# wuqianliang/Diff-Reg

Hardware: AMD Instinct MI355X
Metric: scene-pairs/sec @ 20 denoise steps (N=M=256); IR/FMR parity vs ref (higher is better)
Workload: dtype f32; 1 GPU; cfg2: 3DMatch N=M=256, C=432, 20 denoise steps, max_condition_num=200 (warp active), 256 independent B=1 pairs per pass per GPU as 2 concurrent batch(es), one HIP-graph replay each on its own stream; pairs_per_pass_per_gpu=256, streams=2, denoise_steps=20, N=256, M=256, graph=True, parallelism=pairs sharded over 1 GPU(s)

## Files before the change

diff-reg_amd/csrc/loop.hip:

```cpp
#include "loop_common.h"

namespace dr {

struct LayerWs {
    float *qkv, *att, *mrg, *msg, *hid, *g2;
    size_t T;
    static size_t carve(Carver& c, LayerWs& w, size_t T, int C) {
        w.T = T;
        w.qkv = c.take<float>(T * 3 * C);
        w.att = c.take<float>(T * C);
        w.mrg = c.take<float>(T * C);
        w.msg = c.take<float>(T * C);
        w.hid = c.take<float>(T * 2 * C);
        w.g2 = c.take<float>(T * C);
        return c.off;
    }
};

struct PrepackLayer {
    PgW qkv, merge, mlp0, mlp2;
    const float *lnB1, *lnB2;
};
struct Prepack {
    static constexpr int MAXL = 16;
// ... 56 lines not shown
            if (rc) return rc;
        }
        return pp.head.sub == 2 ? pgemm16w_pack_weights_block(W.src_proj, C, C, C, C, pp.head, 0, st)
                                : pgemm_pack_weights_block(W.src_proj, C, C, C, C, pp.head, 0, st);
    }
};

struct PlanesWs {
    bool on;
    Tok feat0, fa, fb, tgt_l0;
    char *att_img, *msg_img, *hid_img;
    float *att_bnd, *msg_bnd, *hid_bnd;
    char *qkv_img, *kvc_img;
    float *qkv_bnd, *kvc_bnd;
    float* grp_x;
    float* csT;
    size_t qkv_stride;
    size_t side_C, side_att, side_hid;
    void* own_pack;
    float* xk_buf; unsigned* xk_flags; mutable unsigned xk_epoch; unsigned* status;
    static size_t img_bytes(int PN, int PM, int K) { return plane_image_bytes(PN, K) + plane_image_bytes(PM, K); }
    static void carve(Carver& c, PlanesWs& w, const dr_loop_config& cfg, int P, int N, int M) {
        const int C = cfg.C, PN = P * N, PM = P * M, T = PN + PM;
        w.on = planes_wanted(cfg.flags, Prepack::supported(cfg), T);
        if (!w.on) return;
        const int dp = (C / cfg.H + 15) / 16 * 16;
        w.side_C = plane_image_bytes(PN, C); w.side_att = plane_image_bytes(PN, cfg.H * dp); w.side_hid = plane_image_bytes(PN, 2 * C);
        Tok* toks[4] = {&w.feat0, &w.fa, &w.fb, &w.tgt_l0};
        for (Tok* t : toks) { t->f32 = nullptr; t->img = c.take<char>(img_bytes(PN, PM, C)); t->bnd = c.take<float>(T); }
        w.att_img = c.take<char>(img_bytes(PN, PM, cfg.H * dp)); w.att_bnd = c.take<float>(T);
        w.msg_img = c.take<char>(img_bytes(PN, PM, C)); w.msg_bnd = c.take<float>(T);
        w.hid_img = c.take<char>(img_bytes(PN, PM, 2 * C)); w.hid_bnd = c.take<float>(T);
        w.qkv_stride = (img_bytes(PN, PM, cfg.H * dp) + 255) & ~(size_t)255;
        w.qkv_img = c.take<char>(3 * w.qkv_stride); w.qkv_bnd = c.take<float>(3 * (size_t)T);
        w.kvc_img = c.take<char>(2 * w.qkv_stride); w.kvc_bnd = c.take<float>(2 * (size_t)T);
        w.grp_x = c.take<float>(2 * (size_t)P);
        w.csT = c.take<float>((size_t)T * C);
        w.own_pack = c.take<char>(Prepack::carve(nullptr, cfg, nullptr));
        const bool xk = (T + 63) / 64 + 2 <= PG_XK_MAX_RB;
        w.xk_buf = xk ? c.take<float>(pgemm_xk_buf_bytes(pgemm_bn(C)) / 4) : nullptr;
        w.xk_flags = xk ? c.take<unsigned>(pgemm_xk_flag_bytes() / 4) : nullptr;
        w.xk_epoch = 0; w.status = nullptr;
    }
};

static int layer_call(const dr_layer_weights& W, int C, int H, int P, const float* xin, int xr0, int xrows,
                      const float* yin, int yr0, int yrows, const float* cosT, const float* sinT,
                      const uint8_t* tokmask, const Family& f1, const Family* f2, const LayerWs& ws, float* out,
                      hipStream_t st, const float* kv_cached = nullptr, float* kv_store = nullptr, const float* xq_in = nullptr,
                      const float* yk_in = nullptr) {
    const int halfC = C / 2, d = C / H;
    const bool rotary = cosT != nullptr;
    const float* const qin = xq_in ? xq_in : xin;
    const float* const kin = yk_in ? yk_in : yin;
    GemmBatch g;
    memset(&g, 0, sizeof(g));
    auto proj = [&](GemmProblem& p, const float* in, int r0, int rows, const float* Wm, int coloff, bool rot) {
// ... 67 lines not shown
struct PlCtx {
    const Prepack* pp; const PlanesWs* pw; const LayerWs* lw;
    int C, H, P, N, M;
    const float *cosT, *sinT;
    const uint8_t* tokmask;
    int attn_f16;
};
static void xk_assign(const PlanesWs& pw, int C, PgProblem& p, size_t& next, size_t units) {
    if (!pw.xk_buf || next + units > (size_t)PG_XK_MAX_RB) return;
    p.xk_buf = pw.xk_buf + next * (pgemm_xk_buf_bytes(pgemm_bn(C)) / 4 / PG_XK_MAX_RB); p.xk_flags = pw.xk_flags + next * 2; p.xk_cap = (int)units;
    p.xk_epoch = pw.xk_epoch + 1; p.xk_status = pw.status;
    next += units;
}
static size_t xk_wide_units(const PgProblem& p) { return (size_t)(p.rows + 127) / 128 * p.nblk * 2; }

static int layer_call_planes(const PlCtx& X, const dr_layer_weights& W, int l, const Tok& xin, int xs, const Tok& yin, int ys,
                             const Tok& out, const Family& f1, const Family* f2, hipStream_t st, const float* kv_cached = nullptr,
                             float* kv_store = nullptr) {
    const int C = X.C, H = X.H, PN = X.P * X.N, PM = X.P * X.M, halfC = C / 2, d = C / H, nC = C / 16, dp = X.pp->dp;
    const PrepackLayer& L = X.pp->L[l];
    const PlanesWs& pw = *X.pw;
    auto r0 = [&](int side) { return side == SIDE_TGT ? PN : 0; };
    auto nrows = [&](int side) { return side == SIDE_TGT ? PM : PN; };
    auto at = [&](char* img, size_t side_off, int side) { return img + (side == SIDE_TGT ? side_off : 0); };
    PgBatch g;
    size_t xk_next = 0;
    auto reset = [&]() { memset(&g, 0, sizeof(g)); xk_next = 0; };
    auto add = [&]() -> PgProblem& { return g.p[g.n++]; };
    auto for_sides = [&](int mask, auto fn) { for (int side = 1; side <= 2; ++side) if (mask & side) fn(side); };
    auto xk = [&](PgProblem& p, size_t units) { xk_assign(pw, C, p, xk_next, units); };
    int rc;
    bool rc_ok = true;

    const int T = PN + PM, Cq = H * dp, nq = Cq / 16;
    const bool cached = kv_cached != nullptr;
    char* const kv_img = kv_store ? pw.kvc_img : pw.qkv_img + pw.qkv_stride;
    float* const kv_bnd = kv_store ? pw.kvc_bnd : pw.qkv_bnd + T;
    const bool grp_inline = X.N % 128 == 0 && X.M % 128 == 0 && env_knob("DR_LOOP_GRP_INLINE", 1) != 0;
    if (!cached && !grp_inline) {
        for (int side = 1; side <= 2 && rc_ok; ++side)
            if (ys & side) rc_ok = launch_group_max(yin.bnd + r0(side), X.P, side == SIDE_TGT ? X.M : X.N, pw.grp_x + (side == SIDE_TGT ? X.P : 0), st) == DR_OK;
        if (!rc_ok) return DR_ELAUNCH;
    }
    auto proj = [&](const Tok& tin, int side, int b0, int nblk, char* img, float* bnd, int rotm, int grpm) {
        PgProblem& p = add();
        p.A0 = at(tin.img, pw.side_C, side); p.bnd0 = tin.bnd + r0(side); p.nc0 = nC;
        p.W = pgw_blocks(L.qkv, b0, C); p.nblk = nblk; p.rows = nrows(side); p.C = Cq; p.k_alg = C; p.mode = PG_PLANES;
        p.rot_mask = rotm; p.rot_C = C; p.rot_piece_len = d; p.rot_piece_pad = dp; p.scale = 1.f;
        p.cosT = X.cosT + (size_t)r0(side) * halfC; p.sinT = X.sinT + (size_t)r0(side) * halfC;
        p.csT = X.pw->csT + (size_t)r0(side) * halfC * 2;
        p.pimg = at(img, pw.side_att, side); p.p_nct = nq; p.pbnd = bnd + r0(side);
        p.pimg_blk_stride = (long long)pw.qkv_stride; p.pbnd_blk_stride = T;
        p.grp_bnd = grp_inline ? nullptr : pw.grp_x; p.grp_mask = grpm; p.grp_first = side == SIDE_TGT ? X.P : 0; p.grp_rows = side == SIDE_TGT ? X.M : X.N;
        if (p.W.sub == 2) xk(p, xk_wide_units(p));
    };
    reset();
    if (kv_store) {
        for_sides(ys, [&](int side) { proj(yin, side, 1, 2, kv_img, kv_bnd, 1, 3); });
        ++pw.xk_epoch;
        return launch_pgemm(g, st);
    }
    const bool self = xs == ys && xin.img == yin.img && !cached;
    if (self) {
        for_sides(xs, [&](int side) { proj(xin, side, 0, 3, pw.qkv_img, pw.qkv_bnd, 3, 6); });
    } else {
        for_sides(xs, [&](int side) { proj(xin, side, 0, 1, pw.qkv_img, pw.qkv_bnd, 1, 0); });
        if (!cached) for_sides(ys, [&](int side) { proj(yin, side, 1, 2, kv_img, kv_bnd, 1, 3); });
    }
    ++pw.xk_epoch;
    rc = launch_pgemm(g, st);
    if (rc) return rc;

    AttnArgs a;
    memset(&a, 0, sizeof(a));
    a.H = H; a.d = d;
    a.qmask = X.tokmask; a.kmask = X.tokmask;
    a.nseg = X.P; a.q0 = f1.q0; a.qstride = f1.Lq; a.Lq = f1.Lq; a.k0 = f1.k0; a.kstride = f1.Lk; a.Lk = f1.Lk;
    if (f2) { a.nseg2 = X.P; a.q0b = f2->q0; a.qstrideb = f2->Lq; a.Lqb = f2->Lq; a.k0b = f2->k0; a.kstrideb = f2->Lk; a.Lkb = f2->Lk; }
    a.scale = 1.0f / sqrtf((float)d);
    a.pimg[0] = pw.att_img; a.pimg[1] = pw.att_img + pw.side_att; a.p_split = PN; a.p_nct = nq; a.p_dp = dp;
    a.pbnd = pw.att_bnd;
    {
        const char* kimg = cached ? pw.kvc_img : pw.qkv_img + pw.qkv_stride;
        const float* kb = cached ? pw.kvc_bnd : pw.qkv_bnd + T;
        a.qimg[0] = pw.qkv_img; a.qimg[1] = pw.qkv_img + pw.side_att;
        a.kimg[0] = kimg; a.kimg[1] = kimg + pw.side_att;
        a.vimg[0] = kimg + pw.qkv_stride; a.vimg[1] = kimg + pw.qkv_stride + pw.side_att;
        a.qbnd = pw.qkv_bnd; a.kgb = kb; a.vgb = kb + T;
        a.f16_single = X.attn_f16;
    }
    rc = launch_attention(a, st);
    if (rc) return rc;

    reset();
    for_sides(xs, [&](int side) {
        PgProblem& p = add();
        p.A0 = at(pw.att_img, pw.side_att, side); p.bnd0 = pw.att_bnd + r0(side); p.nc0 = H * dp / 16;
        p.W = L.merge; p.nblk = 1; p.rows = nrows(side); p.C = C; p.mode = PG_LN; p.k_alg = C;
        p.gamma = W.norm1_w; p.beta = W.norm1_b; p.lnB = L.lnB1;
        p.pimg = at(pw.msg_img, pw.side_C, side); p.p_nct = nC; p.pbnd = pw.msg_bnd + r0(side);
        xk(p, (size_t)(p.rows + 63) / 64);
    });
    ++pw.xk_epoch;
// ... 23 lines not shown
        xk(p, (size_t)(p.rows + 63) / 64);
    });
    ++pw.xk_epoch;
    return launch_pgemm(g, st);
}

struct DenoiseWs {
    LayerWs lw;
    float *fa, *fb, *cosT, *sinT, *proj, *sim;
    float *tgt_l0, *kv_l1;
    PlanesWs pl;
    const Prepack* pp;
    static void carve(Carver& c, DenoiseWs& w, const dr_loop_config& cfg, int P, int N, int M) {
        const int C = cfg.C;
        const size_t T = (size_t)P * (N + M);
        LayerWs::carve(c, w.lw, T, C);
        PlanesWs::carve(c, w.pl, cfg, P, N, M);
        w.tgt_l0 = c.take<float>(T * C);
        w.kv_l1 = c.take<float>(T * 2 * C);
        w.fa = c.take<float>(T * C);
        w.fb = c.take<float>(T * C);
        w.cosT = c.take<float>(T * (C / 2));
        w.sinT = c.take<float>(T * (C / 2));
        w.proj = c.take<float>(T * C);
        w.sim = c.take<float>((size_t)P * N * M);
        if (w.pl.on) { w.pl.fa.f32 = w.fa; w.pl.fb.f32 = w.fb; w.pl.tgt_l0.f32 = w.tgt_l0; }
    }
};

static int fill_tgt_cache(const dr_loop_config& cfg, const dr_loop_weights& w, int P, int N, int M, const float* feat0,
                          const uint8_t* tokmask, DenoiseWs& ws, hipStream_t st) {
    const int C = cfg.C, H = cfg.H, PN = P * N, PM = P * M;
    const Family self_t{PN, M, PN, M};
    if (ws.pl.on) {
        const PlCtx X{ws.pp, &ws.pl, &ws.lw, C, H, P, N, M, ws.cosT, ws.sinT, tokmask, (cfg.flags & DR_LOOP_ATTN_F16) ? 1 : 0};
        int rc = layer_call_planes(X, w.layers[0], 0, ws.pl.feat0, SIDE_TGT, ws.pl.feat0, SIDE_TGT, ws.pl.tgt_l0, self_t, nullptr, st);
        if (rc || cfg.n_layers < 2) return rc;
        return layer_call_planes(X, w.layers[1], 1, ws.pl.tgt_l0, 0, ws.pl.tgt_l0, SIDE_TGT, ws.pl.tgt_l0, self_t, nullptr, st, nullptr, ws.kv_l1);
    }
    int rc = layer_call(w.layers[0], C, H, P, feat0, PN, PM, feat0, PN, PM, ws.cosT, ws.sinT, tokmask, self_t, nullptr, ws.lw,
                        ws.tgt_l0, st);
    if (rc || cfg.n_layers < 2) return rc;
    return layer_call(w.layers[1], C, H, P, nullptr, 0, 0, ws.tgt_l0, PN, PM, ws.cosT, ws.sinT, tokmask, self_t, nullptr, ws.lw,
                      nullptr, st, nullptr, ws.kv_l1);
}

static int denoiser_and_sim(const dr_loop_config& cfg, const dr_loop_weights& w, int P, int N, int M, const float* feat0,
                            const uint8_t* tokmask, DenoiseWs& ws, const float** final_feats, hipStream_t st,
                            bool use_cache = false) {
    const int C = cfg.C, H = cfg.H, T = P * (N + M), PN = P * N, PM = P * M;
    auto head = [&](const float* feats) {
        return gemm1(feats, C, w.src_proj, nullptr, ws.proj, C, T, C, C, EPI_ROTARY, 1.0f / sqrtf((float)C), nullptr, st, ws.cosT, ws.sinT, C);
    };
    auto sim = [&]() {
        return gemm1(ws.proj, C, ws.proj + (size_t)PN * C, nullptr, ws.sim, M, N, M, C, EPI_NONE, 1.f, nullptr, st, nullptr, nullptr, 0, P,
                     (long long)N * C, (long long)M * C, (long long)N * M);
    };
    if (ws.pl.on) {
        const PlCtx X{ws.pp, &ws.pl, &ws.lw, C, H, P, N, M, ws.cosT, ws.sinT, tokmask, (cfg.flags & DR_LOOP_ATTN_F16) ? 1 : 0};
        const Family self_s{0, N, 0, N}, self_t{PN, M, PN, M}, cross_s{0, N, PN, M}, cross_t{PN, M, 0, N};
        const Tok* cur = &ws.pl.feat0;
        const Tok* bufs[2] = {&ws.pl.fa, &ws.pl.fb};
        int which = 0;
        for (int l = 0; l < cfg.n_layers; ++l) {
            const Tok* nxt = bufs[which];
            int rc;
            if (use_cache && l == 0) {
                nxt = &ws.pl.tgt_l0;
                rc = layer_call_planes(X, w.layers[0], 0, *cur, SIDE_SRC, *cur, SIDE_SRC, *nxt, self_s, nullptr, st);
                if (rc) return rc;
                cur = nxt;
                continue;
            } else if (l % 2 == 0) {
                rc = layer_call_planes(X, w.layers[l], l, *cur, SIDE_BOTH, *cur, SIDE_BOTH, *nxt, self_s, &self_t, st);
                if (rc) return rc;
            } else {
                rc = layer_call_planes(X, w.layers[l], l, *cur, SIDE_SRC, *cur, SIDE_TGT, *nxt, cross_s, nullptr, st,
                                       (use_cache && l == 1) ? ws.kv_l1 : nullptr);
                if (rc) return rc;
                rc = layer_call_planes(X, w.layers[l], l, *cur, SIDE_TGT, *nxt, SIDE_SRC, *nxt, cross_t, nullptr, st);
                if (rc) return rc;
            }
            cur = nxt;
            which ^= 1;
        }
        *final_feats = cur->f32;
        if (env_knob("DR_HEAD_F32", 0)) {
            const int rc = head(cur->f32);
            return rc ? rc : sim();
        }
        PgBatch g;
        memset(&g, 0, sizeof(g));
        size_t xk_next = 0;
        for (int side = 1; side <= 2; ++side) {
            PgProblem& p = g.p[g.n++];
// ... 296 lines not shown
    DR_HIP_CHECK(hipMemcpyAsync(L.feat0, src_feats, PN * C * 4, hipMemcpyDeviceToDevice, st));
    DR_HIP_CHECK(hipMemcpyAsync(L.feat0 + PN * C, tgt_feats, PM * C * 4, hipMemcpyDeviceToDevice, st));
    if (src_mask) {
        DR_HIP_CHECK(hipMemcpyAsync(L.tokmask, src_mask, PN, hipMemcpyDeviceToDevice, st));
        DR_HIP_CHECK(hipMemcpyAsync(L.tokmask + PN, tgt_mask, PM, hipMemcpyDeviceToDevice, st));
    }
    rc = launch_f32_to_f64(x_T, L.x, NM, st);
    if (rc) return rc;
    if (!v4d && P <= 32)
        DR_HIP_CHECK(hipMemsetAsync((char*)L.pmin + pair_min_scratch_bytes(P) - 64 * (size_t)P, 0, 64 * (size_t)P, st));
    Prepack pp;
    rc = planes_begin(*cfg, *w, P, N, M, L.dw, pp, st);
    if (rc) return rc;
    rc = fill_pe(*cfg, *w, P, N, M, s_pcd, nullptr, nullptr, t_pcd, false, true, L.dw, st);
    if (rc) return rc;
    rc = fill_tgt_cache(*cfg, *w, P, N, M, L.feat0, tokmask, L.dw, st);
    if (rc) return rc;

    const float* fin = nullptr;
    SamplerArgs sa;
    memset(&sa, 0, sizeof(sa));
    sa.P = P; sa.N = N; sa.M = M; sa.steps = cfg->steps; sa.alphas_cumprod = cfg->h_alphas_cumprod; sa.times = cfg->h_times;
    sa.sample_rate = cfg->sample_rate; sa.max_condition_num = cfg->max_condition_num; sa.sk_iters = cfg->sk_iters; sa.strict = strict;
    sa.s_pcd = s_pcd; sa.warp_tgt_pcd = t_pcd; sa.src_mask = src_mask; sa.warp_tgt_mask = tgt_mask;
    sa.warp_mflag = mflag; sa.use_mask_len = (v4d || ragged) ? 1 : 0;
    sa.min_shift = !v4d; sa.rsm = rsm; sa.rtm = rtm; sa.dmin = L.dmin; sa.pmin = P <= 32 ? L.pmin : nullptr;
    sa.noise = v4d ? noise : nullptr; sa.bin_score = w->bin_score; sa.trace = trace;
    sa.x = L.x; sa.x_final = x_final; sa.x0 = L.x0; sa.wconf = L.wconf; sa.R = L.R; sa.t = L.t; sa.Rf = L.Rf; sa.tf = L.tf; sa.cond = L.cond; sa.ok = L.ok;
    sa.skws = L.skws; sa.skws_bytes = L.skws_bytes; sa.pws = L.pws; sa.pws_bytes = L.pws_bytes; sa.status = L.status;
    rc = reverse_sampling(sa, [&](const float* Rf, const float* tf) -> int {
        int r = fill_pe(*cfg, *w, P, N, M, s_pcd, Rf, tf, t_pcd, true, false, L.dw, st);
// ... 41 lines not shown
```

diff-reg_amd/csrc/pgemm.h:

```cpp
#pragma once
#include "kernels.h"

namespace dr {

constexpr int PI_BM = 128;
inline size_t plane_image_bytes(size_t rows, int K) { return ((rows + PI_BM - 1) / PI_BM) * (size_t)(K / 16) * (PI_BM * 64); }

struct PgW {
    const char* img;
    const float* cinv;
    const float* wnorm;
    int nct;
    int sub;
};

enum { PG_F32 = 0, PG_PLANES = 1, PG_LN = 2 };

struct PgProblem {
    const char* A0; const char* A1;
    const float* bnd0; const float* bnd1;
    int nc0, nc1;
    PgW W;
    int nblk;
    int rows, C;
// ... 4 lines not shown
    const float* csT;
    int rot_piece_len, rot_piece_pad;
    char* pimg; int p_nct; int p_kc0; float* pbnd;
    long long pimg_blk_stride; long long pbnd_blk_stride;
    const float* grp_bnd; int grp_mask, grp_first, grp_rows;
    int relu;
    const float* gamma; const float* beta; const float* resid; int ldr; const float* bnd_res; const float* lnB;
    int ln_postadd;
    const float* bias; const float* bias_max;
    float* xk_buf; unsigned* xk_flags; unsigned xk_epoch; unsigned* xk_status; int ksplit;
    int xk_cap;
};
constexpr int PG_XK_MAX_RB = 160;
inline size_t pgemm_xk_buf_bytes(int bn) { return (size_t)PG_XK_MAX_RB * 2 * 4 * (bn / 64) * 2 * 64 * 16; }
inline size_t pgemm_xk_flag_bytes() { return (size_t)PG_XK_MAX_RB * 2 * sizeof(unsigned); }
struct PgBatch { PgProblem p[3]; int n; int dbg; };

bool pgemm_shape_ok(int C);
int pgemm_bn(int C);
int launch_pgemm(const PgBatch& g, hipStream_t st);
int pgemm_configure();

size_t pgemm_weight_bytes(int C, int nblk, int nct);
void pgemm_weight_view(void* buf, int C, int nblk, int nct, PgW* view);
int pgemm_pack_weights(const float* W, int nblk, int C, int K, int piece_len, int piece_pad, void* buf, hipStream_t st);
int pgemm_pack_weights_block(const float* W, int C, int K, int piece_len, int piece_pad, const PgW& view, int nb, hipStream_t st, int out_len = 0,
                             int out_pad = 0);
bool pgemm16w_shape_ok(int C);
size_t pgemm16w_weight_bytes(int nblk, int nct);
void pgemm16w_weight_view(void* buf, int nblk, int nct, PgW* view);
int pgemm16w_pack_weights_block(const float* W, int C, int K, int piece_len, int piece_pad, const PgW& view, int nb, hipStream_t st, int out_len = 0,
                                int out_pad = 0);
int launch_group_max(const float* bnd, int ngroups, int grp_rows, float* out, hipStream_t st);

int launch_planes_from_f32(const float* x, int ldx, int rows, int K, char* img, float* bnd, hipStream_t st, const float* bnd_in = nullptr);
int launch_planes_to_f32(const char* img, const float* bnd, int rows, int K, float* out, int ldo, hipStream_t st);
int launch_ln_bound(const float* gamma, const float* beta, int C, float* out, hipStream_t st);
int launch_absmax_blocks(const float* x, int nblk, int n, float* out, hipStream_t st);

}
```

diff-reg_amd/csrc/pgemm.hip:

```cpp
#include <cstdlib>
#include <string.h>
#include <type_traits>
#include "pgemm.h"

namespace dr {
namespace {

typedef float f32x16 __attribute__((ext_vector_type(16)));
typedef float f32x2 __attribute__((ext_vector_type(2)));
typedef _Float16 f16x8 __attribute__((ext_vector_type(8)));
typedef _Float16 f16x2 __attribute__((ext_vector_type(2)));
typedef unsigned u32x4 __attribute__((ext_vector_type(4)));
typedef __attribute__((address_space(3))) void lds_void;
typedef const __attribute__((address_space(1))) void glb_void;

__device__ __forceinline__ void split2(float x0, float x1, unsigned& hi, unsigned& lo) {
    const f32x2 f = {x0, x1};
    const f16x2 h = __builtin_convertvector(f, f16x2);
    hi = __builtin_bit_cast(unsigned, h);
    const f32x2 hf = __builtin_convertvector(h, f32x2);
    const f32x2 r = {x0 - hf.x, x1 - hf.y};
    lo = __builtin_bit_cast(unsigned, __builtin_convertvector(r, f16x2));
}
__device__ __forceinline__ int scale_exp(float m) {
// ... 1412 lines not shown
}

static int launch_pgemm16w(const PgBatch& g, hipStream_t st) {
    int maxt = 0;
    double flops = 0;
    const int mode = g.p[0].mode;
    if (mode != PG_F32 && mode != PG_PLANES) return DR_ENOSUP;
    bool ksplit = env_knob("DR_PG_KSPLIT", 1) != 0 && env_knob("DR_PG_KSPLITW", 1) != 0;
    long tiles = 0;
    for (int i = 0; i < g.n; ++i) {
        const PgProblem& p = g.p[i];
        const long tl_ = (long)((p.rows + 127) / 128) * p.nblk * 2;
        ksplit = ksplit && p.xk_buf && p.xk_flags && tl_ <= p.xk_cap && (p.A1 ? (p.nc0 >= 5 && p.nc1 >= 5) : p.nc0 >= 12);
        tiles += tl_;
    }
    ksplit = ksplit && 2 * tiles <= (long)device_cu_count();
    for (int i = 0; i < g.n; ++i) {
        const PgProblem& p = g.p[i];
        const int nst = p.nc0 + (p.A1 ? p.nc1 : 0);
        if (p.W.sub != 2 || !pgemm16w_shape_ok(p.C) || p.rows < 1 || p.nblk < 1 || p.nc0 < 5 || (p.A1 && p.nc1 < 5) || p.mode != mode) return DR_ENOSUP;
        if (p.W.nct != nst) return DR_EINVAL;
        const int tl = ((p.rows + 127) / 128 + 7) / 8 * 8 * p.nblk * 2 * (ksplit ? 2 : 1);
        maxt = tl > maxt ? tl : maxt;
        flops += 2.0 * p.rows * p.C * p.nblk * (p.k_alg > 0 ? (double)p.k_alg : 16.0 * p.W.nct);
    }
    ProfScope ps(PK_GEMM_SPLIT, flops, st);
    PgBatch gd = g;
    gd.dbg = env_knob("DR_PG_NOEPI", 0);
    for (int i = 0; i < g.n; ++i) gd.p[i].ksplit = ksplit ? 1 : 0;
    const dim3 grid(maxt, g.n);
// ... 1 lines not shown
    else hipLaunchKernelGGL((pgemm16w_kernel<PG_PLANES>), grid, dim3(PgGeomW::NTHR), PgGeomW::SMEM, st, gd);
    DR_LAUNCH_CHECK();
    return DR_OK;
}

int launch_pgemm(const PgBatch& g, hipStream_t st) {
    if (g.n < 1 || g.n > 3) return DR_EINVAL;
    if (g.p[0].W.sub == 2) return launch_pgemm16w(g, st);
    int maxt = 0;
    double flops = 0;
    const int bn = pgemm_bn(g.p[0].C), nst_min = bn == G9::BN ? G9::NST : G7::NST;
    const int half_env = env_knob("DR_PG_HALF", 1);
    const int n_cu = device_cu_count();
    long wg128 = 0;
    for (int i = 0; i < g.n; ++i) wg128 += (long)((g.p[i].rows + 127) / 128) * g.p[i].nblk;
    const bool half = bn == G9::BN || half_env == 2 || (half_env == 1 && wg128 * 100 < (long)n_cu * env_knob("DR_PG_HALF_PCT", 51));
    const int bm = half ? 64 : 128;
    bool ksplit = half && g.p[0].mode == PG_LN && env_knob("DR_PG_KSPLIT", 1) != 0;
    long wg64 = 0;
    for (int i = 0; i < g.n; ++i) {
        const PgProblem& p = g.p[i];
        const long rb64 = (p.rows + 63) / 64;
        ksplit = ksplit && p.xk_buf && p.xk_flags && p.nblk == 1 && !p.A1 && p.nc0 / 2 >= nst_min && rb64 <= p.xk_cap;
        wg64 += rb64;
    }
    ksplit = ksplit && 2 * wg64 <= (long)n_cu;
    for (int i = 0; i < g.n; ++i) {
        const PgProblem& p = g.p[i];
        if (!pgemm_shape_ok(p.C) || pgemm_bn(p.C) != bn || p.rows < 1 || p.nblk < 1 || p.nc0 < 1 || p.nc0 + (p.A1 ? p.nc1 : 0) < nst_min) return DR_ENOSUP;
        if (p.W.nct != p.nc0 + (p.A1 ? p.nc1 : 0)) return DR_EINVAL;
// ... 107 lines not shown
    DR_LAUNCH_CHECK();
    return DR_OK;
}

__global__ __launch_bounds__(256) void group_max_kernel(const float* __restrict__ bnd, int ngroups, int grp_rows, float* __restrict__ out) {
    const int g = blockIdx.x * 4 + (threadIdx.x >> 6), lane = threadIdx.x & 63;
    if (g >= ngroups) return;
    float m = 0.f;
    for (int r = lane; r < grp_rows; r += 64) m = fmaxf(m, bnd[(size_t)g * grp_rows + r]);
    m = wave_max(m);
    if (lane == 0) out[g] = m;
}
int launch_group_max(const float* bnd, int ngroups, int grp_rows, float* out, hipStream_t st) {
    if (ngroups < 1) return DR_OK;
    hipLaunchKernelGGL(group_max_kernel, dim3((ngroups + 3) / 4), dim3(256), 0, st, bnd, ngroups, grp_rows, out);
    DR_LAUNCH_CHECK();
    return DR_OK;
}

int launch_planes_from_f32(const float* x, int ldx, int rows, int K, char* img, float* bnd, hipStream_t st, const float* bnd_in) {
    if (K % 16 || K > 1024 || ldx % 4 || ((uintptr_t)x & 15)) return DR_ENOSUP;
    if (rows < 1) return DR_OK;
    hipLaunchKernelGGL(planes_from_f32_kernel, dim3((rows + 3) / 4), dim3(256), 0, st, x, ldx, rows, K, img, bnd, bnd_in);
    DR_LAUNCH_CHECK();
    return DR_OK;
}
int launch_planes_to_f32(const char* img, const float* bnd, int rows, int K, float* out, int ldo, hipStream_t st) {
    if (K % 16) return DR_ENOSUP;
    if (rows < 1) return DR_OK;
    hipLaunchKernelGGL(planes_to_f32_kernel, dim3((rows + 3) / 4), dim3(256), 0, st, img, bnd, rows, K, out, ldo);
// ... 145 lines not shown
    if (p.mode != PG_F32 && !p.pimg && !p.out) return DR_EINVAL;
    if (p.mode == PG_PLANES && !p.pimg) return DR_EINVAL;
    g.n = 1;
    if (a->split_workspace) {
        const int bn = a->weight_layout == DR_PL_LAYOUT_WIDE ? 576 : pgemm_bn(a->C);
        if (a->split_workspace_bytes < dr_plane_split_workspace_bytes(a->C) || ((uintptr_t)a->split_workspace & 15)) return DR_EWORKSPACE;
        char* w = (char*)a->split_workspace;
        DR_HIP_CHECK(hipMemsetAsync(w, 0, 16 + pgemm_xk_flag_bytes(), (hipStream_t)stream));
        p.xk_status = (unsigned*)w; p.xk_flags = (unsigned*)(w + 16); p.xk_buf = (float*)(w + 16 + ((pgemm_xk_flag_bytes() + 255) & ~(size_t)255));
        p.xk_epoch = 1; p.xk_cap = PG_XK_MAX_RB;
        (void)bn;
    }
    return launch_pgemm(g, (hipStream_t)stream);
}

size_t dr_plane_split_workspace_bytes(int C) {
    if (C < 16 || C > 576) return 0;
    return 16 + ((pgemm_xk_flag_bytes() + 255) & ~(size_t)255) + pgemm_xk_buf_bytes(576);
}

int dr_plane_split_status(void* split_workspace, void* stream, int clear) {
    if (!split_workspace) return DR_EINVAL;
    return sinkhorn_call_status((unsigned*)split_workspace, (hipStream_t)stream, clear != 0);
}

}
```

diff-reg_amd/diffreg_hip/lib.py:

```python
import ctypes
import os

import torch

_HERE = os.path.dirname(os.path.abspath(__file__))
LIB_PATH = os.path.join(_HERE, "libdiffreg_hip.so")

if not os.path.exists(LIB_PATH):
    raise ImportError("libdiffreg_hip.so is missing (%s): run `python __graft_entry__.py build` or "
                      "`make -C diff-reg_amd/csrc`" % LIB_PATH)

_lib = ctypes.CDLL(LIB_PATH)

c_int, c_size_t, c_void_p, c_char_p, c_double, c_float = (ctypes.c_int, ctypes.c_size_t, ctypes.c_void_p,
                                                          ctypes.c_char_p, ctypes.c_double, ctypes.c_float)

SIGNATURES = {
    "dr_version": (c_int, []),
    "dr_strerror": (c_char_p, [c_int]),
    "dr_last_hip_error": (c_char_p, []),
    "dr_sinkhorn_workspace_bytes": (c_size_t, [c_int, c_int, c_int, c_int, c_int]),
    "dr_sinkhorn_f32": (c_int, [c_int, c_int, c_int, c_void_p, c_void_p, c_void_p, c_void_p, c_int, c_int,
                                c_void_p, c_void_p, c_size_t, c_void_p]),
    "dr_sinkhorn_f16": (c_int, [c_int, c_int, c_int, c_void_p, c_void_p, c_void_p, c_void_p, c_int, c_int, c_void_p, c_void_p]),
# ... 84 lines not shown
    "dr_plane_image_bytes": (c_size_t, [c_int, c_int]),
    "dr_planes_from_f32": (c_int, [c_int, c_int, c_void_p, c_int, c_void_p, c_void_p, c_void_p]),
    "dr_planes_from_f32_bounded": (c_int, [c_int, c_int, c_void_p, c_int, c_void_p, c_void_p, c_void_p, c_void_p]),
    "dr_attention_planes": (c_int, [c_int] * 5 + [c_void_p] * 10 + [c_void_p]),
    "dr_attention_planes_f16": (c_int, [c_int] * 5 + [c_void_p] * 10 + [c_void_p]),
    "dr_planes_to_f32": (c_int, [c_int, c_int, c_void_p, c_void_p, c_void_p, c_int, c_void_p]),
    "dr_plane_weight_bytes": (c_size_t, [c_int, c_int, c_int, c_int, c_int]),
    "dr_pack_weight_planes_f32": (c_int, [c_int, c_int, c_int, c_int, c_int, c_void_p, c_void_p, c_void_p]),
    "dr_plane_weight_bytes_wide": (c_size_t, [c_int, c_int, c_int, c_int, c_int]),
    "dr_plane_split_workspace_bytes": (c_size_t, [c_int]),
    "dr_plane_split_status": (c_int, [c_void_p, c_void_p, c_int]),
    "dr_pack_weight_planes_wide_f32": (c_int, [c_int, c_int, c_int, c_int, c_int, c_void_p, c_void_p, c_void_p]),
    "dr_ln_bound_f32": (c_int, [c_int, c_void_p, c_void_p, c_void_p, c_void_p]),
    "dr_linear_planes_f32": (c_int, [ctypes.POINTER(PlanesLinear), c_void_p]),
    "dr_bias_max_f32": (c_int, [c_int, c_int, c_void_p, c_void_p, c_void_p]),
    "dr_loop2d3d_prepack_bytes": (c_size_t, [ctypes.POINTER(Loop2D3DConfig)]),
    "dr_loop2d3d_prepack": (c_int, [ctypes.POINTER(Loop2D3DConfig), ctypes.POINTER(FusionWeights), c_void_p, c_size_t, c_void_p]),
    "dr_gemm_nt_batched_f32": (c_int, [c_int, c_int, c_int, c_int, c_void_p, ctypes.c_longlong, c_void_p, ctypes.c_longlong, c_void_p, ctypes.c_longlong,
                                       c_float, c_void_p]),
    "dr_linear_ex_f32": (c_int, [c_int, c_int, c_int, c_void_p, c_int, c_void_p, c_void_p, c_void_p, c_int, c_int, c_float, c_void_p]),
    "dr_kpconv_gather_f32": (c_int, [c_int, c_int, c_int, c_int, c_int, c_void_p, c_void_p, c_void_p, c_void_p, c_void_p, c_float,
                                     c_void_p, c_int, c_void_p]),
    "dr_kpconv_gather_mode_f32": (c_int, [c_int, c_int, c_int, c_int, c_int, c_void_p, c_void_p, c_void_p, c_void_p, c_void_p, c_float,
                                          c_int, c_int, c_void_p, c_int, c_void_p]),
    "dr_kpconv_gather_backward_mode_f32": (c_int, [c_int, c_int, c_int, c_int, c_int, c_void_p, c_void_p, c_void_p, c_void_p, c_void_p, c_float,
                                                   c_int, c_int, c_void_p, c_int, c_void_p, c_void_p]),
    "dr_col_stats_workspace_bytes": (c_size_t, [c_int, c_int]),
    "dr_col_stats_f32": (c_int, [c_int, c_int, c_void_p, c_int, c_void_p, c_void_p, c_void_p, c_size_t, c_void_p]),
    "dr_norm_apply_f32": (c_int, [c_int, c_int, c_void_p, c_int, c_void_p, c_void_p, c_void_p, c_int, c_void_p, c_void_p, c_float,
                                  c_int, c_void_p, c_int, c_void_p]),
# ... 309 lines not shown
    a.cos_t, a.sin_t, a.rot_mask, a.rot_C, a.scale = dp(cos_t), dp(sin_t), rot_mask, rot_C, scale
    a.out_image, a.out_image_k, a.out_k0, a.out_bound = dp(out_image), out_image_k, out_k0, dp(out_bound)
    a.relu = 1 if relu else 0
    a.gamma, a.beta, a.resid, a.ldr, a.bound_resid, a.ln_bound = dp(gamma), dp(beta), dp(resid), ldr, dp(bound_resid), dp(lnb)
    bmax = None
    if bias is not None:
        bias = bias.contiguous().float()
        bmax = torch.empty(nblk, device=bias.device)
        check(_lib.dr_bias_max_f32(nblk, C, ptr(bias), ptr(bmax), stream_of(a0)))
    a.bias, a.bias_max, a.ln_postadd = dp(bias), dp(bmax), 1 if ln_postadd else 0
    a.weight_layout = 1 if wide else 0
    a.split_workspace, a.split_workspace_bytes = dp(split_ws), (split_ws.numel() if split_ws is not None else 0)
    check(_lib.dr_linear_planes_f32(ctypes.byref(a), stream_of(a0)))


def plane_split_workspace(C, device):
    return torch.empty(_lib.dr_plane_split_workspace_bytes(C), dtype=torch.uint8, device=device)


def plane_split_status(split_ws, clear=True):
    check(_lib.dr_plane_split_status(ptr(split_ws), stream_of(split_ws), 1 if clear else 0))


def scatter_rows(src, src_index, dst_index, dst, validate=True, status=None):
    ensure_init()
    src = src.contiguous().float()
    si = src_index.to(device=src.device, dtype=torch.int64).contiguous()
    di = dst_index.to(device=src.device, dtype=torch.int64).contiguous()
    assert dst.is_contiguous() and dst.dtype == torch.float32 and dst.shape[-1] == src.shape[-1] and dst.device == src.device
    assert si.numel() == di.numel()
# ... 1102 lines not shown
```

include/diffreg_hip.h:

```cpp
#ifndef DIFFREG_HIP_H
#define DIFFREG_HIP_H

#include <stddef.h>
#include <stdint.h>

#ifdef __cplusplus
extern "C" {
#endif

#define DR_OK 0
#define DR_EINVAL (-1)
#define DR_ELAUNCH (-2)
#define DR_ENOSUP (-3)
#define DR_EWORKSPACE (-4)
#define DR_ETIMEOUT (-5)

#define DR_ABI_VERSION 700
int dr_version(void);
const char* dr_strerror(int code);
const char* dr_last_hip_error(void);

int dr_device_status(void* stream, int clear);

#define DR_SK_OUT_CONF 0x0
// ... 59 lines not shown
    float* out; int ldo; int blk_stride;
    const float* cos_t; const float* sin_t; int rot_mask; int rot_C; float scale;
    void* out_image; int out_image_k; int out_k0; float* out_bound;
    int relu;
    const float* gamma; const float* beta; const float* resid; int ldr; const float* bound_resid; const float* ln_bound;
    const float* bias; const float* bias_max;
    int ln_postadd;
    int weight_layout;
    void* split_workspace; size_t split_workspace_bytes;
} dr_planes_linear;
size_t dr_plane_split_workspace_bytes(int C);
int dr_plane_split_status(void* split_workspace, void* stream, int clear);
#define DR_PL_LAYOUT_BLOCK 0
#define DR_PL_LAYOUT_WIDE 1
int dr_linear_planes_f32(const dr_planes_linear* args, void* stream);
int dr_bias_max_f32(int nblk, int n, const float* bias, float* out, void* stream);

int dr_gemm_nt_batched_f32(int nbatch, int rows, int ncols, int K, const float* A, long long stride_a, const float* W, long long stride_w, float* out,
                           long long stride_o, float scale, void* stream);

int dr_linear_ex_f32(int rows, int ncols, int K, const float* x, int lda, const float* W, const float* bias, float* out,
                     int ldo, int epilogue, float scale, void* stream);

int dr_kpconv_gather_f32(int Nq, int Ns, int H, int Cin, int K, const float* q_pts, const float* s_pts,
                         const int64_t* neighb_inds, const float* x, const float* kernel_points, float extent,
                         float* weighted, int ld_weighted, void* stream);
#define DR_KP_CONSTANT 0
#define DR_KP_LINEAR 1
#define DR_KP_GAUSSIAN 2
int dr_kpconv_gather_mode_f32(int Nq, int Ns, int H, int Cin, int K, const float* q_pts, const float* s_pts, const int64_t* neighb_inds,
// ... 392 lines not shown
```

Baseline: 1194 pairs/s.

## Hoist step-invariant layer-0 source projections and layer-1 target queries out of denoise loop

Precomputes, once per pass, the layer-0 source-side Q/K projections (pre-rotary, in f32), the V projection image, and the layer-1 target query image, because these depend only on step-invariant features. Each denoise step then applies rotary and plane-packing through a new lightweight kernel, or reuses the cached images directly, instead of rerunning the projection GEMMs. The cache lives in the layer workspace, which is reused, and is gated by an env knob. A wg_as override keeps the GEMM tile heuristics matched to the original problem size. The cost is extra workspace aliasing and more code paths.

```diff
diff --git a/diff-reg_amd/csrc/loop.hip b/diff-reg_amd/csrc/loop.hip
--- a/diff-reg_amd/csrc/loop.hip
+++ b/diff-reg_amd/csrc/loop.hip
@@ -94,6 +94,10 @@
     char *qkv_img, *kvc_img;
     float *qkv_bnd, *kvc_bnd;
     float* grp_x;
+    bool hoist;
+    float* pre0;
+    char* v0_img; float *v0_bnd, *grp0;
+    char* q1_img; float* q1_bnd;
     float* csT;
     size_t qkv_stride;
     size_t side_C, side_att, side_hid;
@@ -115,12 +119,21 @@
         w.qkv_img = c.take<char>(3 * w.qkv_stride); w.qkv_bnd = c.take<float>(3 * (size_t)T);
         w.kvc_img = c.take<char>(2 * w.qkv_stride); w.kvc_bnd = c.take<float>(2 * (size_t)T);
         w.grp_x = c.take<float>(2 * (size_t)P);
+        w.hoist = false;
         w.csT = c.take<float>((size_t)T * C);
         w.own_pack = c.take<char>(Prepack::carve(nullptr, cfg, nullptr));
         const bool xk = (T + 63) / 64 + 2 <= PG_XK_MAX_RB;
         w.xk_buf = xk ? c.take<float>(pgemm_xk_buf_bytes(pgemm_bn(C)) / 4) : nullptr;
         w.xk_flags = xk ? c.take<unsigned>(pgemm_xk_flag_bytes() / 4) : nullptr;
         w.xk_epoch = 0; w.status = nullptr;
+    }
+    static void carve_hoist(PlanesWs& w, char* mem, size_t bytes, const dr_loop_config& cfg, int P, int N, int M) {
+        const int PN = P * N, PM = P * M, T = PN + PM, Cq = cfg.H * ((cfg.C / cfg.H + 15) / 16 * 16);
+        Carver c(mem);
+        w.pre0 = c.take<float>((size_t)PN * 2 * Cq);
+        w.v0_img = c.take<char>(plane_image_bytes(PN, Cq)); w.v0_bnd = c.take<float>(PN); w.grp0 = c.take<float>(P);
+        w.q1_img = c.take<char>(plane_image_bytes(PM, Cq)); w.q1_bnd = c.take<float>(T);
+        w.hoist = c.off <= bytes && env_knob("DR_LOOP_HOIST", 1) != 0;
     }
 };
 
@@ -218,9 +231,15 @@
 }
 static size_t xk_wide_units(const PgProblem& p) { return (size_t)(p.rows + 127) / 128 * p.nblk * 2; }
 
+struct PlHoist {
+    bool l0_fill = false;
+    bool l0_use = false;
+    bool q1_fill = false;
+    bool q1_use = false;
+};
 static int layer_call_planes(const PlCtx& X, const dr_layer_weights& W, int l, const Tok& xin, int xs, const Tok& yin, int ys,
                              const Tok& out, const Family& f1, const Family* f2, hipStream_t st, const float* kv_cached = nullptr,
-                             float* kv_store = nullptr) {
+                             float* kv_store = nullptr, const PlHoist& hz = PlHoist()) {
     const int C = X.C, H = X.H, PN = X.P * X.N, PM = X.P * X.M, halfC = C / 2, d = C / H, nC = C / 16, dp = X.pp->dp;
     const PrepackLayer& L = X.pp->L[l];
     const PlanesWs& pw = *X.pw;
@@ -241,7 +260,7 @@
     char* const kv_img = kv_store ? pw.kvc_img : pw.qkv_img + pw.qkv_stride;
     float* const kv_bnd = kv_store ? pw.kvc_bnd : pw.qkv_bnd + T;
     const bool grp_inline = X.N % 128 == 0 && X.M % 128 == 0 && env_knob("DR_LOOP_GRP_INLINE", 1) != 0;
-    if (!cached && !grp_inline) {
+    if (!cached && !grp_inline && !hz.l0_fill && !hz.l0_use && !hz.q1_fill) {
         for (int side = 1; side <= 2 && rc_ok; ++side)
             if (ys & side) rc_ok = launch_group_max(yin.bnd + r0(side), X.P, side == SIDE_TGT ? X.M : X.N, pw.grp_x + (side == SIDE_TGT ? X.P : 0), st) == DR_OK;
         if (!rc_ok) return DR_ELAUNCH;
@@ -264,16 +283,53 @@
         ++pw.xk_epoch;
         return launch_pgemm(g, st);
     }
+    const int rbS = (PN + 127) / 128, rbT = (PM + 127) / 128;
+    if (hz.l0_fill) {
+        rc = launch_group_max(xin.bnd, X.P, X.N, pw.grp0, st);
+        if (rc) return rc;
+        proj(xin, SIDE_SRC, 0, 2, pw.qkv_img, pw.qkv_bnd, 0, 0);
+        g.p[0].mode = PG_F32; g.p[0].pimg = nullptr; g.p[0].pbnd = nullptr;
+        g.p[0].out = pw.pre0; g.p[0].ldo = 2 * Cq; g.p[0].blk_stride = Cq;
+        g.wg_as = 3 * rbS;
+        ++pw.xk_epoch;
+        rc = launch_pgemm(g, st);
+        if (rc) return rc;
+        reset();
+        proj(xin, SIDE_SRC, 2, 1, pw.v0_img, pw.v0_bnd, 0, 1);
+        g.p[0].grp_bnd = pw.grp0; g.p[0].grp_first = 0;
+        g.wg_as = 3 * rbS;
+        ++pw.xk_epoch;
+        return launch_pgemm(g, st);
+    }
+    if (hz.q1_fill) {
+        proj(xin, SIDE_TGT, 0, 1, pw.qkv_img, pw.qkv_bnd, 1, 0);
+        g.p[0].pimg = pw.q1_img; g.p[0].pbnd = pw.q1_bnd + PN;
+        g.wg_as = rbT + 2 * rbS;
+        ++pw.xk_epoch;
+        return launch_pgemm(g, st);
+    }
     const bool self = xs == ys && xin.img == yin.img && !cached;
-    if (self) {
-        for_sides(xs, [&](int side) { proj(xin, side, 0, 3, pw.qkv_img, pw.qkv_bnd, 3, 6); });
+    if (hz.l0_use) {
+        RotImgArgs r;
+        memset(&r, 0, sizeof(r));
+        r.x = pw.pre0; r.ldx = 2 * Cq; r.x_blk = Cq; r.rows = PN; r.C = Cq; r.nblk = 2;
+        r.csT = pw.csT; r.rot_mask = 3; r.rot_C = C; r.rot_piece_len = d; r.rot_piece_pad = dp; r.scale = 1.f;
+        r.bnd0 = xin.bnd; r.wnorm = L.qkv.wnorm; r.wide_form = L.qkv.sub == 2; r.grp_bnd = pw.grp0; r.grp_mask = 2; r.grp_first = 0; r.grp_rows = X.N;
+        r.pimg = pw.qkv_img; r.p_nct = nq; r.pbnd = pw.qkv_bnd; r.pimg_blk_stride = (long long)pw.qkv_stride; r.pbnd_blk_stride = T;
+        rc = launch_rot_images(r, st);
+        if (rc) return rc;
     } else {
-        for_sides(xs, [&](int side) { proj(xin, side, 0, 1, pw.qkv_img, pw.qkv_bnd, 1, 0); });
-        if (!cached) for_sides(ys, [&](int side) { proj(yin, side, 1, 2, kv_img, kv_bnd, 1, 3); });
-    }
-    ++pw.xk_epoch;
-    rc = launch_pgemm(g, st);
-    if (rc) return rc;
+        if (self) {
+            for_sides(xs, [&](int side) { proj(xin, side, 0, 3, pw.qkv_img, pw.qkv_bnd, 3, 6); });
+        } else {
+            if (!hz.q1_use) for_sides(xs, [&](int side) { proj(xin, side, 0, 1, pw.qkv_img, pw.qkv_bnd, 1, 0); });
+            else g.wg_as = rbT + 2 * rbS;
+            if (!cached) for_sides(ys, [&](int side) { proj(yin, side, 1, 2, kv_img, kv_bnd, 1, 3); });
+        }
+        ++pw.xk_epoch;
+        rc = launch_pgemm(g, st);
+        if (rc) return rc;
+    }
 
     AttnArgs a;
     memset(&a, 0, sizeof(a));
@@ -291,6 +347,8 @@
         a.kimg[0] = kimg; a.kimg[1] = kimg + pw.side_att;
         a.vimg[0] = kimg + pw.qkv_stride; a.vimg[1] = kimg + pw.qkv_stride + pw.side_att;
         a.qbnd = pw.qkv_bnd; a.kgb = kb; a.vgb = kb + T;
+        if (hz.l0_use) { a.vimg[0] = pw.v0_img; a.vgb = pw.v0_bnd; }
+        if (hz.q1_use) { a.qimg[1] = pw.q1_img; a.qbnd = pw.q1_bnd; }
         a.f16_single = X.attn_f16;
     }
     rc = launch_attention(a, st);
@@ -344,8 +402,11 @@
     static void carve(Carver& c, DenoiseWs& w, const dr_loop_config& cfg, int P, int N, int M) {
         const int C = cfg.C;
         const size_t T = (size_t)P * (N + M);
+        const size_t lw_begin = align256(c.off);
         LayerWs::carve(c, w.lw, T, C);
+        const size_t lw_end = c.off;
         PlanesWs::carve(c, w.pl, cfg, P, N, M);
+        if (w.pl.on) PlanesWs::carve_hoist(w.pl, c.base ? c.base + lw_begin : nullptr, lw_end - lw_begin, cfg, P, N, M);
         w.tgt_l0 = c.take<float>(T * C);
         w.kv_l1 = c.take<float>(T * 2 * C);
         w.fa = c.take<float>(T * C);
@@ -358,15 +419,22 @@
     }
 };
 
-static int fill_tgt_cache(const dr_loop_config& cfg, const dr_loop_weights& w, int P, int N, int M, const float* feat0,
+static int fill_step_invariants(const dr_loop_config& cfg, const dr_loop_weights& w, int P, int N, int M, const float* feat0,
                           const uint8_t* tokmask, DenoiseWs& ws, hipStream_t st) {
     const int C = cfg.C, H = cfg.H, PN = P * N, PM = P * M;
     const Family self_t{PN, M, PN, M};
     if (ws.pl.on) {
         const PlCtx X{ws.pp, &ws.pl, &ws.lw, C, H, P, N, M, ws.cosT, ws.sinT, tokmask, (cfg.flags & DR_LOOP_ATTN_F16) ? 1 : 0};
         int rc = layer_call_planes(X, w.layers[0], 0, ws.pl.feat0, SIDE_TGT, ws.pl.feat0, SIDE_TGT, ws.pl.tgt_l0, self_t, nullptr, st);
+        if (rc == DR_OK && ws.pl.hoist) {
+            PlHoist hz; hz.l0_fill = true;
+            rc = layer_call_planes(X, w.layers[0], 0, ws.pl.feat0, SIDE_SRC, ws.pl.feat0, SIDE_SRC, ws.pl.tgt_l0, Family{0, N, 0, N}, nullptr, st, nullptr, nullptr, hz);
+        }
         if (rc || cfg.n_layers < 2) return rc;
-        return layer_call_planes(X, w.layers[1], 1, ws.pl.tgt_l0, 0, ws.pl.tgt_l0, SIDE_TGT, ws.pl.tgt_l0, self_t, nullptr, st, nullptr, ws.kv_l1);
+        rc = layer_call_planes(X, w.layers[1], 1, ws.pl.tgt_l0, 0, ws.pl.tgt_l0, SIDE_TGT, ws.pl.tgt_l0, self_t, nullptr, st, nullptr, ws.kv_l1);
+        if (rc || !ws.pl.hoist) return rc;
+        PlHoist hz; hz.q1_fill = true;
+        return layer_call_planes(X, w.layers[1], 1, ws.pl.tgt_l0, SIDE_TGT, ws.pl.tgt_l0, 0, ws.pl.tgt_l0, self_t, nullptr, st, nullptr, nullptr, hz);
     }
     int rc = layer_call(w.layers[0], C, H, P, feat0, PN, PM, feat0, PN, PM, ws.cosT, ws.sinT, tokmask, self_t, nullptr, ws.lw,
                         ws.tgt_l0, st);
@@ -397,7 +465,8 @@
             int rc;
             if (use_cache && l == 0) {
                 nxt = &ws.pl.tgt_l0;
-                rc = layer_call_planes(X, w.layers[0], 0, *cur, SIDE_SRC, *cur, SIDE_SRC, *nxt, self_s, nullptr, st);
+                PlHoist hz; hz.l0_use = ws.pl.hoist;
+                rc = layer_call_planes(X, w.layers[0], 0, *cur, SIDE_SRC, *cur, SIDE_SRC, *nxt, self_s, nullptr, st, nullptr, nullptr, hz);
                 if (rc) return rc;
                 cur = nxt;
                 continue;
@@ -408,7 +477,8 @@
                 rc = layer_call_planes(X, w.layers[l], l, *cur, SIDE_SRC, *cur, SIDE_TGT, *nxt, cross_s, nullptr, st,
                                        (use_cache && l == 1) ? ws.kv_l1 : nullptr);
                 if (rc) return rc;
-                rc = layer_call_planes(X, w.layers[l], l, *cur, SIDE_TGT, *nxt, SIDE_SRC, *nxt, cross_t, nullptr, st);
+                PlHoist hz; hz.q1_use = use_cache && l == 1 && ws.pl.hoist;
+                rc = layer_call_planes(X, w.layers[l], l, *cur, SIDE_TGT, *nxt, SIDE_SRC, *nxt, cross_t, nullptr, st, nullptr, nullptr, hz);
                 if (rc) return rc;
             }
             cur = nxt;
@@ -735,7 +805,7 @@
     if (rc) return rc;
     rc = fill_pe(*cfg, *w, P, N, M, s_pcd, nullptr, nullptr, t_pcd, false, true, L.dw, st);
     if (rc) return rc;
-    rc = fill_tgt_cache(*cfg, *w, P, N, M, L.feat0, tokmask, L.dw, st);
+    rc = fill_step_invariants(*cfg, *w, P, N, M, L.feat0, tokmask, L.dw, st);
     if (rc) return rc;
 
     const float* fin = nullptr;
diff --git a/diff-reg_amd/csrc/pgemm.h b/diff-reg_amd/csrc/pgemm.h
--- a/diff-reg_amd/csrc/pgemm.h
+++ b/diff-reg_amd/csrc/pgemm.h
@@ -42,7 +42,7 @@
 constexpr int PG_XK_MAX_RB = 160;
 inline size_t pgemm_xk_buf_bytes(int bn) { return (size_t)PG_XK_MAX_RB * 2 * 4 * (bn / 64) * 2 * 64 * 16; }
 inline size_t pgemm_xk_flag_bytes() { return (size_t)PG_XK_MAX_RB * 2 * sizeof(unsigned); }
-struct PgBatch { PgProblem p[3]; int n; int dbg; };
+struct PgBatch { PgProblem p[3]; int n; int dbg; int wg_as; };
 
 bool pgemm_shape_ok(int C);
 int pgemm_bn(int C);
@@ -61,6 +61,18 @@
                                 int out_pad = 0);
 int launch_group_max(const float* bnd, int ngroups, int grp_rows, float* out, hipStream_t st);
 
+struct RotImgArgs {
+    const float* x; int ldx, x_blk;
+    int rows, C, nblk;
+    const float* csT; int rot_mask, rot_C, rot_piece_len, rot_piece_pad; float scale;
+    const float* bnd0;
+    const float* wnorm;
+    int wide_form;
+    const float* grp_bnd; int grp_mask, grp_first, grp_rows;
+    char* pimg; int p_nct; float* pbnd; long long pimg_blk_stride, pbnd_blk_stride;
+};
+int launch_rot_images(const RotImgArgs& a, hipStream_t st);
+
 int launch_planes_from_f32(const float* x, int ldx, int rows, int K, char* img, float* bnd, hipStream_t st, const float* bnd_in = nullptr);
 int launch_planes_to_f32(const char* img, const float* bnd, int rows, int K, float* out, int ldo, hipStream_t st);
 int launch_ln_bound(const float* gamma, const float* beta, int C, float* out, hipStream_t st);
diff --git a/diff-reg_amd/csrc/pgemm.hip b/diff-reg_amd/csrc/pgemm.hip
--- a/diff-reg_amd/csrc/pgemm.hip
+++ b/diff-reg_amd/csrc/pgemm.hip
@@ -1450,6 +1450,7 @@
         ksplit = ksplit && p.xk_buf && p.xk_flags && tl_ <= p.xk_cap && (p.A1 ? (p.nc0 >= 5 && p.nc1 >= 5) : p.nc0 >= 12);
         tiles += tl_;
     }
+    if (g.wg_as > 0) tiles = 2L * g.wg_as;
     ksplit = ksplit && 2 * tiles <= (long)device_cu_count();
     for (int i = 0; i < g.n; ++i) {
         const PgProblem& p = g.p[i];
@@ -1481,6 +1482,7 @@
     const int n_cu = device_cu_count();
     long wg128 = 0;
     for (int i = 0; i < g.n; ++i) wg128 += (long)((g.p[i].rows + 127) / 128) * g.p[i].nblk;
+    if (g.wg_as > 0) wg128 = g.wg_as;
     const bool half = bn == G9::BN || half_env == 2 || (half_env == 1 && wg128 * 100 < (long)n_cu * env_knob("DR_PG_HALF_PCT", 51));
     const int bm = half ? 64 : 128;
     bool ksplit = half && g.p[0].mode == PG_LN && env_knob("DR_PG_KSPLIT", 1) != 0;
@@ -1618,6 +1620,73 @@
 int launch_group_max(const float* bnd, int ngroups, int grp_rows, float* out, hipStream_t st) {
     if (ngroups < 1) return DR_OK;
     hipLaunchKernelGGL(group_max_kernel, dim3((ngroups + 3) / 4), dim3(256), 0, st, bnd, ngroups, grp_rows, out);
+    DR_LAUNCH_CHECK();
+    return DR_OK;
+}
+
+__global__ __launch_bounds__(256) void rot_images_kernel(RotImgArgs A) {
+    const int t = threadIdx.x, row = blockIdx.x * 64 + (t >> 2), j = t & 3;
+    const int kc = 2 * blockIdx.y + (j >> 1), hh = j & 1, col0 = kc * 16 + hh * 8;
+    if (row >= A.rows || col0 >= A.C) return;
+    const int halfC = A.rot_C >> 1, rpad = A.rot_piece_pad, rlen = A.rot_piece_len;
+    float4 tb[2];
+    if (A.rot_mask) {
+        const float* pp = A.csT + (size_t)row * halfC * 2;
+#pragma unroll
+        for (int i = 0; i < 2; ++i) {
+            int col = min(col0 + 4 * i, A.C - 4);
+            if (rpad > 0) { const int hq = col / rpad; col = hq * rlen + min(col - hq * rpad, rlen - 4); }
+            if (col >= A.rot_C) col %= A.rot_C;
+            const float4 cs = *reinterpret_cast<const float4*>(pp + 2 * (col >> 1));
+            tb[i] = make_float4(cs.x, cs.z, cs.y, cs.w);
+        }
+    }
+    const float b0 = A.bnd0[row], scale = A.scale;
+    const int rl = row & 127, swz = (rl >> 2) & 3;
+    typedef unsigned u32x4v __attribute__((ext_vector_type(4)));
+    for (int nb = 0; nb < A.nblk; ++nb) {
+        const bool rot = (A.rot_mask >> nb) & 1;
+        const float* xp = A.x + (size_t)row * A.ldx + (size_t)nb * A.x_blk + col0;
+        float4 v[2] = {*reinterpret_cast<const float4*>(xp), *reinterpret_cast<const float4*>(xp + 4)};
+#pragma unroll
+        for (int i = 0; i < 2; ++i) {
+            float4 x = v[i];
+            if (rot) {
+                const float x0 = x.x, x1 = x.y, x2 = x.z, x3 = x.w;
+                x.x = __builtin_fmaf(x0, tb[i].x, -(x1 * tb[i].z));
+                x.z = __builtin_fmaf(x2, tb[i].y, -(x3 * tb[i].w));
+                if (A.wide_form) {
+                    x.y = __builtin_fmaf(x0, tb[i].z, x1 * tb[i].x);
+                    x.w = __builtin_fmaf(x2, tb[i].w, x3 * tb[i].y);
+                } else {
+                    x.y = __builtin_fmaf(x1, tb[i].x, x0 * tb[i].z);
+                    x.w = __builtin_fmaf(x3, tb[i].y, x2 * tb[i].w);
+                }
+            }
+            x.x *= scale; x.y *= scale; x.z *= scale; x.w *= scale;
+            v[i] = x;
+        }
+        const float bin = ((A.grp_mask >> nb) & 1) ? A.grp_bnd[A.grp_first + row / A.grp_rows] : fmaxf(b0, 0.f);
+        const float bound = (bin * A.wnorm[nb] + 0.f) * (rot ? 1.41421366f : 1.f) * fabsf(scale);
+        if (col0 == 0) A.pbnd[(size_t)nb * A.pbnd_blk_stride + row] = bound;
+        const float sc = pow2i(scale_exp(bound));
+        unsigned h0, l0, h1, l1, h2, l2, h3, l3;
+        split2(v[0].x * sc, v[0].y * sc, h0, l0); split2(v[0].z * sc, v[0].w * sc, h1, l1);
+        split2(v[1].x * sc, v[1].y * sc, h2, l2); split2(v[1].z * sc, v[1].w * sc, h3, l3);
+        const u32x4v hi = {h0, h1, h2, h3}, lo = {l0, l1, l2, l3};
+        char* const rowp = A.pimg + (size_t)nb * A.pimg_blk_stride + (((size_t)(row >> 7) * A.p_nct + kc) * 128 + rl) * 64;
+        __builtin_nontemporal_store(hi, reinterpret_cast<u32x4v*>(rowp + ((hh ^ swz) << 4)));
+        __builtin_nontemporal_store(lo, reinterpret_cast<u32x4v*>(rowp + (((2 + hh) ^ swz) << 4)));
+    }
+}
+int launch_rot_images(const RotImgArgs& a, hipStream_t st) {
+    if (a.rows < 1) return DR_OK;
+    if (a.nblk < 1 || a.nblk > 3 || a.C < 16 || a.C % 16 || a.C / 16 > a.p_nct || a.ldx % 4 || a.x_blk % 4 || ((uintptr_t)a.x & 15) || !a.x || !a.bnd0 ||
+        !a.wnorm || !a.pimg || !a.pbnd || ((uintptr_t)a.pimg & 15) || (a.grp_mask && (!a.grp_bnd || a.grp_rows < 1)))
+        return DR_EINVAL;
+    if (a.rot_mask && (!a.csT || ((uintptr_t)a.csT & 15) || a.rot_C % 4 || a.rot_piece_len % 4 || a.rot_piece_pad % 4)) return DR_EINVAL;
+    ProfScope ps(PK_PE, (double)a.rows * (8.0 * a.nblk * a.C + (a.rot_mask ? 4.0 * a.rot_C : 0.0)), st);
+    hipLaunchKernelGGL(rot_images_kernel, dim3((a.rows + 63) / 64, (a.C / 16 + 1) / 2), dim3(256), 0, st, a);
     DR_LAUNCH_CHECK();
     return DR_OK;
 }
@@ -1793,6 +1862,28 @@
     return launch_pgemm(g, (hipStream_t)stream);
 }
 
+int dr_rotary_planes_f32(int rows, int C, int nblk, const float* x, int ldx, int x_blk, const float* cs_t, int rot_mask, int rot_C, float scale,
+                         const float* bound0, const void* packed, int k, int weight_layout, void* out_image, long long image_blk_stride,
+                         float* out_bound, long long bound_blk_stride, void* stream) {
+    if (rows < 0 || nblk < 1 || nblk > 3 || !x || !bound0 || !packed || !out_image || !out_bound || k < 16 || k % 16 || ldx < C || C < 16 || C % 16 ||
+        (rot_mask && (!cs_t || rot_C < 4))) return DR_EINVAL;
+    PgW v;
+    if (weight_layout == DR_PL_LAYOUT_WIDE) {
+        if (!pgemm16w_shape_ok(C)) return DR_EINVAL;
+        pgemm16w_weight_view((void*)packed, nblk, k / 16, &v);
+    } else if (weight_layout == DR_PL_LAYOUT_BLOCK) {
+        if (!pgemm_shape_ok(C)) return DR_EINVAL;
+        pgemm_weight_view((void*)packed, C, nblk, k / 16, &v);
+    } else return DR_EINVAL;
+    RotImgArgs r;
+    memset(&r, 0, sizeof(r));
+    r.x = x; r.ldx = ldx; r.x_blk = x_blk; r.rows = rows; r.C = C; r.nblk = nblk;
+    r.csT = cs_t; r.rot_mask = rot_mask; r.rot_C = rot_C; r.scale = scale;
+    r.bnd0 = bound0; r.wnorm = v.wnorm; r.wide_form = v.sub == 2;
+    r.pimg = (char*)out_image; r.p_nct = C / 16; r.pbnd = out_bound; r.pimg_blk_stride = image_blk_stride; r.pbnd_blk_stride = bound_blk_stride;
+    return launch_rot_images(r, (hipStream_t)stream);
+}
+
 size_t dr_plane_split_workspace_bytes(int C) {
     if (C < 16 || C > 576) return 0;
     return 16 + ((pgemm_xk_flag_bytes() + 255) & ~(size_t)255) + pgemm_xk_buf_bytes(576);
diff --git a/diff-reg_amd/diffreg_hip/lib.py b/diff-reg_amd/diffreg_hip/lib.py
--- a/diff-reg_amd/diffreg_hip/lib.py
+++ b/diff-reg_amd/diffreg_hip/lib.py
@@ -122,6 +122,8 @@
     "dr_ln_bound_f32": (c_int, [c_int, c_void_p, c_void_p, c_void_p, c_void_p]),
     "dr_linear_planes_f32": (c_int, [ctypes.POINTER(PlanesLinear), c_void_p]),
     "dr_bias_max_f32": (c_int, [c_int, c_int, c_void_p, c_void_p, c_void_p]),
+    "dr_rotary_planes_f32": (c_int, [c_int, c_int, c_int, c_void_p, c_int, c_int, c_void_p, c_int, c_int, c_float, c_void_p, c_void_p, c_int, c_int,
+                                     c_void_p, ctypes.c_longlong, c_void_p, ctypes.c_longlong, c_void_p]),
     "dr_loop2d3d_prepack_bytes": (c_size_t, [ctypes.POINTER(Loop2D3DConfig)]),
     "dr_loop2d3d_prepack": (c_int, [ctypes.POINTER(Loop2D3DConfig), ctypes.POINTER(FusionWeights), c_void_p, c_size_t, c_void_p]),
     "dr_gemm_nt_batched_f32": (c_int, [c_int, c_int, c_int, c_int, c_void_p, ctypes.c_longlong, c_void_p, ctypes.c_longlong, c_void_p, ctypes.c_longlong,
@@ -461,6 +463,13 @@
     check(_lib.dr_linear_planes_f32(ctypes.byref(a), stream_of(a0)))
 
 
+def rotary_planes(x, x_blk, C, nblk, cs_t, rot_mask, rot_C, b0, packed, k, out_image, image_blk_stride, out_bound, bound_blk_stride, scale=1.0,
+                  wide=False):
+    ensure_init()
+    check(_lib.dr_rotary_planes_f32(x.shape[0], C, nblk, ptr(x), x.stride(0), x_blk, ptr(cs_t), rot_mask, rot_C, scale, ptr(b0), ptr(packed), k,
+                                    1 if wide else 0, ptr(out_image), image_blk_stride, ptr(out_bound), bound_blk_stride, stream_of(x)))
+
+
 def plane_split_workspace(C, device):
     return torch.empty(_lib.dr_plane_split_workspace_bytes(C), dtype=torch.uint8, device=device)
 
diff --git a/include/diffreg_hip.h b/include/diffreg_hip.h
--- a/include/diffreg_hip.h
+++ b/include/diffreg_hip.h
@@ -97,6 +97,9 @@
 #define DR_PL_LAYOUT_BLOCK 0
 #define DR_PL_LAYOUT_WIDE 1
 int dr_linear_planes_f32(const dr_planes_linear* args, void* stream);
+int dr_rotary_planes_f32(int rows, int C, int nblk, const float* x, int ldx, int x_blk, const float* cs_t, int rot_mask, int rot_C, float scale,
+                         const float* bound0, const void* packed, int k, int weight_layout, void* out_image, long long image_blk_stride,
+                         float* out_bound, long long bound_blk_stride, void* stream);
 int dr_bias_max_f32(int nblk, int n, const float* bias, float* out, void* stream);
 
 int dr_gemm_nt_batched_f32(int nbatch, int rows, int ncols, int K, const float* A, long long stride_a, const float* W, long long stride_w, float* out,
```

Measured after the change: 1212 pairs/s (median of 6 runs). 1.01x the previous value.
